# fnothaft/spark-bam

Measured on AMD Instinct MI355X. Metric: compressed BAM GB/s for compute-splits + full-check (whole node, 1/2/4/8 GPU), higher is better.
Workload: dtype u8

## Files before the change

### spark-bam_amd/csrc/sbam_inflate.hip

```cpp
#include <type_traits>

#include "sbam_internal.h"
#include "sbam_resolve_core.h"

namespace sbam {

#define SB_DEV __device__ __forceinline__

enum : int32_t { INF_OK = 0, INF_SHORT = 1, INF_DATA = 2, INF_OVERFLOW = 3 };

constexpr uint32_t kTokPad = 0x7fffu;
constexpr uint32_t kTokDist = 0x8000u;

SB_DEV uint64_t tok_region(int64_t uoff, int64_t b) {
  return (((uint64_t)uoff + 15) & ~15ull) + 32ull * (uint64_t)b;
}
SB_DEV int32_t tok_region_cap(int32_t us) { return (us + 16) / 2; }
SB_DEV uint64_t tok_arena_need(int32_t us) { return ((uint64_t)(2 * us + 32) + 15) & ~15ull; }

constexpr int kDecThreads = 256;
constexpr int kRows = 80;
constexpr int kLitSorted = 0;
constexpr int kClTab = 0;
constexpr int kLensLitRow = 32;
// ... 726 lines not shown
  bool over = false;
  uint32_t code = 0;
  sfor<1, 16>([&](auto I) {
    constexpr int l = decltype(I)::value;
    const uint32_t k = uni(cnt[l]);
    left = 2 * left - (int)k;
    over |= left < 0;
    c.lim[l] = (code + k) << (15 - l);
    c.base[l] = acc - (int32_t)code;
    offs[l] = acc;
    acc += (int32_t)k;
    code = (code + k) << 1;
  });
  c.lim[0] = 0;
  c.base[0] = 0;
  if (over || left != 0) return false;
  int32_t run[16];
  sfor<1, 16>([&](auto I) { run[decltype(I)::value] = 0; });
  for (int c0 = 0; c0 < nsym; c0 += 64) {
    const int s = c0 + lane;
    const uint32_t l = s < nsym ? lens[off + s] : 0u;
    sfor<1, 16>([&](auto I) {
      constexpr int ll = decltype(I)::value;
      const uint64_t m = __ballot(l == (uint32_t)ll);
      const uint32_t below = __builtin_amdgcn_mbcnt_hi((uint32_t)(m >> 32), __builtin_amdgcn_mbcnt_lo((uint32_t)m, 0u));
      if (l == (uint32_t)ll) sorted[off + offs[ll] + run[ll] + (int)below] = (uint16_t)s;
      run[ll] += __popcll(m);
    });
  }
  __syncthreads();
  for (int e = lane; e < (1 << R); e += 64) {
    const uint32_t v = (__builtin_bitreverse32((uint32_t)e) >> (32 - R)) << (15 - R);
    if (v < c.lim[R]) {
      const uint32_t l = canon_len<R>(c, v);
      L.tab[2 * e + DIST] = sym_entry(sorted[off + (int)(v >> (15 - l)) + canon_base<R>(c, l)], l, DIST);
    }
  }
  const uint32_t P0 = c.lim[R] >> (15 - R);
  const int npre = (1 << R) - (int)P0;
  uint16_t *own = reinterpret_cast<uint16_t *>(L.win);
  uint32_t *pinfo = L.win + 256;
  static_assert(wd::kLitSub <= 512 && 256 + 512 <= wd::kWinDw - wd::kScratchDw, "sub-table scratch in the window");
  int next = 0;
  for (int j0 = 0; j0 < npre; j0 += 64) {
    const int j = j0 + lane;
    const uint32_t P = P0 + (uint32_t)j;
    uint32_t sb = 0, sz = 0;
    if (j < npre) {
      sb = canon_len(c, ((P + 1) << (15 - R)) - 1) - R;
      sz = 1u << sb;
    }
    const uint32_t incl = wave_incl_scan(sz);
    const int my = next + (int)(incl - sz);
    if (j < npre && my + (int)sz <= subcap) {
      L.tab[2 * (__builtin_bitreverse32(P) >> (32 - R)) + DIST] =
          (wd::K_SUBP << 8) | sb | ((uint32_t)(4 * (suboff + my)) << 16);
      pinfo[j] = (uint32_t)my | (sb << 16);
      for (uint32_t k = 0; k < sz; k++) own[my + (int)k] = (uint16_t)j;
    }
    next += (int)__shfl(incl, 63);
  }
  __syncthreads();
  if (next <= subcap) {
    for (int e = lane; e < next; e += 64) {
      const int j = own[e];
      const uint32_t info = pinfo[j], sb = info >> 16, P = P0 + (uint32_t)j, k = (uint32_t)e - (info & 0xffffu);
      const uint32_t v = (P << (15 - R)) | ((__builtin_bitreverse32(k) >> (32 - sb)) << (15 - R - sb));
      const uint32_t l = canon_len(c, v);
      L.tab[suboff + e] = sym_entry(sorted[off + (int)(v >> (15 - l)) + canon_base(c, l)], l, DIST);
    }
  }
  __syncthreads();
  return next <= subcap;
}

SB_DEV uint32_t lds_addr(const void *p) {
  return (uint32_t)(uintptr_t)(const __attribute__((address_space(3))) void *)p;
}

typedef const __attribute__((address_space(3))) uint32_t *lds_u32;
SB_DEV lds_u32 win_at(const uint32_t *wp, int pos) {
  uint32_t a;
  asm("v_lshl_add_u32 %0, %1, 2, %2" : "=v"(a) : "v"((uint32_t)pos >> 5), "s"(lds_addr(wp)));
  return reinterpret_cast<lds_u32>((uintptr_t)a);
}
SB_DEV uint32_t tsym(const WaveLds &L, uint32_t lo0, uint32_t hi, int &pos, uint32_t st4, uint32_t &v) {
  using namespace wd;
  const uint32_t lo = __builtin_amdgcn_alignbit(hi, lo0, (uint32_t)pos);
  static_assert(kLitRoot == 9 && kDistRoot == 9, "interleaved 9-bit roots");
  const char *tb = reinterpret_cast<const char *>(L.tab);
  uint32_t e = *reinterpret_cast<const uint32_t *>(tb + (((lo << 3) & 0xff8u) | st4));
  if (((e >> 8) & 0xffu) == K_SUBP)
    e = *reinterpret_cast<const uint32_t *>(tb + (e >> 16) + 4u * __builtin_amdgcn_ubfe(lo, 9u, e));
  const uint32_t n = e & 15u, x = (e >> 4) & 15u;
  v = (e >> 16) + __builtin_amdgcn_ubfe(lo, n, x);
  pos += (int)(n + x);
  return (e >> 8) & 0xffu;
}
SB_DEV uint32_t wsym(const uint32_t *wp, const WaveLds &L, int &pos, uint32_t st4, uint32_t &v) {
  const lds_u32 q = win_at(wp, pos);
  return tsym(L, q[0], q[1], pos, st4, v);
}

struct HBits {
  uint64_t bb;
  int bc, rp, pos;
  SB_DEV void init(const uint32_t *win, int wq, int p) {
    const int rel = p - wq, w = rel >> 5, sh = rel & 31;
    bb = (((uint64_t)uni(win[w]) | ((uint64_t)uni(win[w + 1]) << 32)) >> sh);
    bc = 64 - sh;
    rp = w + 2;
    pos = p;
  }
  SB_DEV uint32_t get(const uint32_t *win, int n) {
    if (bc < 32) {
      bb |= (uint64_t)uni(win[rp]) << bc;
      bc += 32;
      rp++;
    }
    const uint32_t v = (uint32_t)bb & ((1u << n) - 1u);
    bb >>= n;
    bc -= n;
    pos += n;
    return v;
  }
};

SB_DEV void wave_stage(uint32_t *win, const uint32_t *base, int64_t base_dw, int wq_dw, int64_t lim_dw) {
  constexpr int kN = (wd::kWinDw + 255) / 256;
  const int lane = (int)threadIdx.x;
  __syncthreads();
  {
    const int64_t last = lim_dw - 4 - base_dw;
#pragma unroll
    for (int k = 0; k < kN; k++) {
      const int i = lane * 4 + 256 * k;
      if (i < wd::kWinDw) {
        int64_t o = (int64_t)wq_dw + i;
        o = o > last ? last : o;
        __builtin_amdgcn_global_load_lds(base + o, win + 256 * k, 16, 0, 0);
      }
    }
    asm volatile("s_waitcnt vmcnt(0)" ::: "memory");
  }
  __syncthreads();
}
struct SegResult {
  uint32_t tok, byt, exit;
  int stop;
  bool bad;
};

#ifdef SBAM_WAVE_STATS
constexpr int kWaveStats = 40;
__device__ unsigned long long g_wave_stats[kWaveStats];
#define WMARK(slot) do { const uint64_t t_ = __builtin_amdgcn_s_memtime(); ws_[slot] += t_ - wt_; wt_ = t_; } while (0)
#define WADD(slot, v) ws_[slot] += (v)
extern "C" int sbam_debug_wave_stats(unsigned long long *out, int reset) {
  if (hipMemcpyFromSymbol(out, HIP_SYMBOL(g_wave_stats), sizeof(g_wave_stats)) != hipSuccess) return -1;
  if (reset) {
    static const unsigned long long z[kWaveStats] = {0};
    if (hipMemcpyToSymbol(HIP_SYMBOL(g_wave_stats), z, sizeof(z)) != hipSuccess) return -1;
  }
  return 0;
}
#else
#define WMARK(slot) do {} while (0)
#define WADD(slot, v) do {} while (0)
#endif
#ifdef SBAM_WAVE_STATS
#define RMARK(k) do { const uint64_t t_ = __builtin_amdgcn_s_memtime(); rs_[k] += t_ - rt_; rt_ = t_; } while (0)
#else
#define RMARK(k) do {} while (0)
#endif

constexpr int kMaxStored = 64;
constexpr int64_t kTokDone = -2;

SB_DEV bool stored_copy(const uint8_t *__restrict__ d, int64_t a, int dlen, int bitp, int32_t us,
                        uint8_t *__restrict__ ob, int64_t U0, uint32_t *seg) {
  const int lane = (int)threadIdx.x;
  int n = 0, o = 0;
  if ((bitp + 3 + 7) / 8 > dlen) return false;
  bool fin;
  {
    const uint32_t h3 = (uint32_t)d[a + (bitp >> 3)] | (uint32_t)d[a + (bitp >> 3) + 1] << 8;
    const uint32_t hb = (h3 >> (bitp & 7)) & 7u;
    if (((hb >> 1) & 3u) != 0u) return false;
    fin = (hb & 1u) != 0u;
    bitp += 3;
  }
  for (;;) {
    const int byp = (bitp + 7) >> 3;
    if (byp + 4 > dlen || n == kMaxStored) return false;
    const uint32_t len = (uint32_t)d[a + byp] | (uint32_t)d[a + byp + 1] << 8;
    const uint32_t nlen = (uint32_t)d[a + byp + 2] | (uint32_t)d[a + byp + 3] << 8;
    if ((len ^ 0xffffu) != nlen) return false;
    const int dat = byp + 4;
    if (dat + (int)len > dlen) return false;
    if (lane == 0) {
      seg[2 * n] = (uint32_t)o;
      seg[2 * n + 1] = (uint32_t)dat;
    }
    n++;
    o += (int)len;
    if (o > us) return false;
    if (fin) break;
    const int nb = dat + (int)len;
    if (nb >= dlen) return false;
    const uint32_t h3 = d[a + nb];
    if (((h3 >> 1) & 3u) != 0u) return false;
    fin = (h3 & 1u) != 0u;
    bitp = nb * 8 + 3;
  }
  if (o != us) return false;
  __syncthreads();
  for (int j = 0; j < n; j++) {
    const int o0 = (int)seg[2 * j], o1 = j + 1 < n ? (int)seg[2 * j + 2] : us;
    const uint8_t *src = d + a + (int)seg[2 * j + 1] - o0;
    const int c0 = o0 + (int)((16 - ((U0 + o0) & 15)) & 15), c1 = o1 - (int)((U0 + o1) & 15);
    if (c0 + 16 <= c1) {
      int x = c0 + 16 * lane;
      for (; x + 3 * 1024 + 16 <= c1; x += 4 * 1024) {
        const u32x4 v0 = __builtin_nontemporal_load(reinterpret_cast<const u32x4 *>(src + x));
        const u32x4 v1 = __builtin_nontemporal_load(reinterpret_cast<const u32x4 *>(src + x + 1024));
        const u32x4 v2 = __builtin_nontemporal_load(reinterpret_cast<const u32x4 *>(src + x + 2048));
        const u32x4 v3 = __builtin_nontemporal_load(reinterpret_cast<const u32x4 *>(src + x + 3072));
        *reinterpret_cast<u32x4 *>(ob + x) = v0;
        *reinterpret_cast<u32x4 *>(ob + x + 1024) = v1;
        *reinterpret_cast<u32x4 *>(ob + x + 2048) = v2;
        *reinterpret_cast<u32x4 *>(ob + x + 3072) = v3;
      }
      for (; x + 16 <= c1; x += 1024)
        *reinterpret_cast<u32x4 *>(ob + x) = __builtin_nontemporal_load(reinterpret_cast<const u32x4 *>(src + x));
      if (lane < c0 - o0) ob[o0 + lane] = src[o0 + lane];
      if (lane < o1 - c1) ob[c1 + lane] = src[c1 + lane];
    } else {
      for (int x = o0 + lane; x < o1; x += 64) ob[x] = src[x];
    }
  }
  return true;
}

__global__ __launch_bounds__(64, 4) void k_inflate_wave(const uint8_t *__restrict__ d, int64_t D, BlockTable bt,
                                                     TokPool tp, int32_t *__restrict__ status,
                                                     int32_t *__restrict__ found, int32_t *__restrict__ slow,
                                                     unsigned int *nslow) {
  using namespace wd;
  __shared__ __attribute__((aligned(16))) WaveLds L;
  const int lane = (int)threadIdx.x;
  const int64_t b = blockIdx.x;
  const int64_t st0 = bt.start[b];
  const int32_t hs = bt.hsize[b], cs = bt.csize[b], us = bt.usize[b];
  const int32_t dlen = cs - hs - 8;
  if (us == 0 || us < 0 || us > 65536 || dlen < 0 || st0 + hs + dlen > D) {
    if (lane == 0) {
      status[b] = us == 0 ? INF_OK : INF_DATA;
      found[b] = 0;
    }
    return;
  }
  const int64_t a = st0 + hs;
  const int64_t base_dw = (a >> 4) << 2;
  const uint32_t *base = reinterpret_cast<const uint32_t *>(d) + base_dw;
  const int64_t lim_dw = (D + kCompPad) >> 2;
  const int skip = (int)(a - base_dw * 4) * 8;
  const int pend = skip + 8 * dlen;
  uint8_t *reg = tp.main + tok_region(bt.uoff[b], b);
  int32_t tcap = tok_region_cap(us);
  uint8_t *lens = L.lens();
  int pos = skip;
  int out = 0, ntok = 0;
  bool ok = true, stored = false;
#ifdef SBAM_WAVE_STATS
  uint64_t ws_[32] = {0};
  uint64_t wt_ = __builtin_amdgcn_s_memtime();
  const uint64_t wt0_ = wt_;
#endif

  for (bool fin = false; ok && !fin;) {
    int wq = (pos >> 7) << 7;
    wave_stage(L.win, base, base_dw, wq >> 5, lim_dw);
    WMARK(12);
    if (pos + 3 > pend) { ok = false; break; }
    HBits h;
    h.init(L.win, wq, pos);
    fin = h.get(L.win, 1) != 0;
    const uint32_t type = h.get(L.win, 2);
    int hlit = 288, hdist = 32;
    if (type == 1) {
      for (int i = lane; i < 320; i += 64)
        lens[i] = i < 144 ? 8 : i < 256 ? 9 : i < 280 ? 7 : i < 288 ? 8 : 5;
    } else if (type == 2) {
      hlit = (int)h.get(L.win, 5) + 257;
      hdist = (int)h.get(L.win, 5) + 1;
      const int hclen = (int)h.get(L.win, 4) + 4;
      if (hlit > 286 || hdist > 30) { ok = false; break; }
      uint64_t clp = 0;
      for (int i = 0; i < 19; i++)
        if (i < hclen) clp |= (uint64_t)h.get(L.win, 3) << (3 * kClOrder[i]);
      const uint32_t lsym = lane < 19 ? (uint32_t)(clp >> (3 * lane)) & 7u : 0u;
      int left = 1;
      bool over = false;
      uint32_t lim7[8], base7[8], code = 0;
      int acc = 0;
#pragma unroll
      for (int l = 1; l <= 7; l++) {
// ... 374 lines not shown
        if (lane < (nb - nb16) / 2)
          reinterpret_cast<uint16_t *>(nreg + nb16)[lane] = reinterpret_cast<const uint16_t *>(reg + nb16)[lane];
        if (lane == 0) tp.base[b] = (int64_t)at;
        reg = nreg;
        tcap = 1 << 30;
      }
      bool tail = false;
      uint32_t tail_ti = 0, tail_st = 0;
      uint32_t r_lo = 0, r_hi = 0, r_tb = 0;
      if (act) {
        uint32_t start = __shfl_up(nxt, 1);
        if (lane == 0) start = S;
        uint32_t ti = (uint32_t)ntok + (itok - my_tok);
        auto run = [&](uint32_t st, int endp) {
          uint32_t st4 = (st >> 7) & 4u;
          int rp = (int)(st >> 10);
          while (rp < endp) {
            uint32_t v;
            const uint32_t kind = wsym(wp, L, rp, st4, v);
            if (kind == K_SPEC) break;
            st4 = kind == K_LEN ? 4u : 0u;
            *reinterpret_cast<uint16_t *>(reg + 2 * ti) = (uint16_t)v;
            ti++;
          }
        };
        WMARK(24);
        run(start, mode == kModeF ? seg_end : mode == kModeR ? (int)rjP : 0);
        WMARK(25);
        const uint32_t lo = mode == kModeR ? rjs : 0u;
        const uint32_t n = mode == kModeA ? res.tok : mode == kModeR ? res.tok - rjtk : 0u;
        const uint32_t hi = mode == kModeF ? 0u : min(lo + n, (uint32_t)kTR);
        const uint32_t tb = ti - lo;
        r_lo = lo;
        r_hi = hi;
        r_tb = tb;
        static_assert(kTR == 80, "one asm operand per register token dword");
        asm volatile("" : "+v"(tr[0]), "+v"(tr[1]), "+v"(tr[2]), "+v"(tr[3]), "+v"(tr[4]), "+v"(tr[5]), "+v"(tr[6]), "+v"(tr[7]), "+v"(tr[8]), "+v"(tr[9]), "+v"(tr[10]), "+v"(tr[11]), "+v"(tr[12]), "+v"(tr[13]), "+v"(tr[14]), "+v"(tr[15]), "+v"(tr[16]), "+v"(tr[17]), "+v"(tr[18]), "+v"(tr[19]), "+v"(tr[20]), "+v"(tr[21]), "+v"(tr[22]), "+v"(tr[23]), "+v"(tr[24]), "+v"(tr[25]), "+v"(tr[26]), "+v"(tr[27]), "+v"(tr[28]), "+v"(tr[29]), "+v"(tr[30]), "+v"(tr[31]), "+v"(tr[32]), "+v"(tr[33]), "+v"(tr[34]), "+v"(tr[35]), "+v"(tr[36]), "+v"(tr[37]), "+v"(tr[38]), "+v"(tr[39]));
        {
          const uint32_t par = tb & 1u;
          uint8_t *pa = reg + 2 * ((int64_t)ti - (int64_t)lo);
          if (par && lo == 0 && hi > 0) *reinterpret_cast<uint16_t *>(pa) = (uint16_t)tr[0];
          u32x4a *pv = reinterpret_cast<u32x4a *>(pa + 2 * par);
          uint32_t *pw = reinterpret_cast<uint32_t *>(pa + 2 * par);
          auto dw = [&](auto Q) {
            constexpr int q = decltype(Q)::value;
            const uint32_t nx = q + 1 < kTR / 2 ? tr[q + 1 < kTR / 2 ? q + 1 : q] : 0u;
            return par ? __builtin_amdgcn_alignbit(nx, tr[q], 16) : tr[q];
          };
          sfor<0, kTR / 8>([&](auto C) {
            constexpr int c = decltype(C)::value;
            const uint32_t a0 = dw(std::integral_constant<int, 4 * c>{}), a1 = dw(std::integral_constant<int, 4 * c + 1>{});
            const uint32_t a2 = dw(std::integral_constant<int, 4 * c + 2>{}), a3 = dw(std::integral_constant<int, 4 * c + 3>{});
            const uint32_t t0 = par + 8 * c;
            if (t0 >= lo && t0 + 8 <= hi) {
              pv[c] = u32x4a{a0, a1, a2, a3};
            } else if (t0 + 8 > lo && t0 < hi) {
              const uint32_t a[4] = {a0, a1, a2, a3};
#pragma unroll
              for (int k = 0; k < 4; k++) {
                const uint32_t u0 = t0 + 2 * k;
                const bool in0 = u0 >= lo && u0 < hi, in1 = u0 + 1 >= lo && u0 + 1 < hi;
                uint16_t *ph = reinterpret_cast<uint16_t *>(pw + 4 * c + k);
                if (in0 && in1) pw[4 * c + k] = a[k];
                else if (in0) ph[0] = (uint16_t)a[k];
                else if (in1) ph[1] = (uint16_t)(a[k] >> 16);
              }
            }
          });
        }
        WMARK(26);
        WMARK(27);
        tail = mode != kModeF && lo + n > (uint32_t)kTR;
        tail_st = lo <= (uint32_t)kTR ? stR : rjP << 10;
        tail_ti = lo <= (uint32_t)kTR ? tb + kTR : ti;
      }
      if (tail) {
        uint32_t st4 = (tail_st >> 7) & 4u, ti = tail_ti;
        int rp = (int)(tail_st >> 10);
        while (rp < seg_end) {
          uint32_t v;
          const uint32_t kind = wsym(wp, L, rp, st4, v);
          if (kind == K_SPEC) break;
          st4 = kind == K_LEN ? 4u : 0u;
          *reinterpret_cast<uint16_t *>(reg + 2 * ti) = (uint16_t)v;
          ti++;
        }
      }
      (void)r_lo;
      (void)r_hi;
      (void)r_tb;
      WMARK(28);
      out += (int)tot_byt;
      ntok += (int)tot_tok;
      if (f < 64) {
        pos = (int)(uni((uint32_t)__shfl(res.exit, f)) >> 10);
        break;
      }
      S = uni((uint32_t)__shfl(nxt, 63));
    }
  }
  if (ok && out != us) ok = false;
#ifdef SBAM_WAVE_STATS
  ws_[8] = __builtin_amdgcn_s_memtime() - wt0_;
  if (lane == 0)
    for (int i = 0; i < 29; i++) atomicAdd(&g_wave_stats[i], (unsigned long long)ws_[i]);
#endif
  if (lane == 0) {
    if (ok) {
      status[b] = INF_OK;
      found[b] = us;
    } else if (stored) {
      slow[bt.n + atomicAdd(nslow + 3, 1u)] = (int32_t)b;
    } else {
      slow[atomicAdd(nslow, 1u)] = (int32_t)b;
    }
  }
}

__global__ __launch_bounds__(64) void k_inflate_stored(const uint8_t *__restrict__ d, BlockTable bt, TokPool tp,
                                                      uint8_t *__restrict__ out, int32_t *__restrict__ status,
                                                      int32_t *__restrict__ found, int32_t *__restrict__ slow,
                                                      unsigned int *nslow) {
  __shared__ uint32_t seg[2 * kMaxStored];
  const unsigned n = nslow[3];
  for (unsigned i = blockIdx.x; i < n; i += gridDim.x) {
    const int64_t b = slow[bt.n + i];
    const int64_t a = bt.start[b] + bt.hsize[b], U0 = bt.uoff[b];
    const int32_t dlen = bt.csize[b] - bt.hsize[b] - 8, us = bt.usize[b];
    if (stored_copy(d, a, dlen, 0, us, out + U0, U0, seg)) {
      if (threadIdx.x == 0) {
        tp.base[b] = kTokDone;
        status[b] = INF_OK;
        found[b] = us;
      }
    } else if (threadIdx.x == 0) {
      slow[atomicAdd(nslow, 1u)] = (int32_t)b;
    }
    __syncthreads();
  }
}

namespace rs {
constexpr int kSpan = 1024;
constexpr int kFlush = 1024;
}
namespace rc = sbam_resolve;

template <int RB>
struct RingGeom {
  static constexpr uint32_t kRing = 1u << RB, kMask = kRing - 1u, kDw = kRing / 4u, kDwMask = kDw - 1u;
  static constexpr uint32_t kMirror = 8u;
  static constexpr int kNear = (int)kRing - rs::kSpan - 264;
  static_assert(kNear >= rs::kSpan + rs::kFlush + 272, "far sources are in HBM");
  static_assert((int)kRing > rs::kSpan + 260 + rs::kFlush, "slots are flushed before reuse");
};

template <class G>
SB_DEV void ring_or1(uint32_t *ring, uint32_t i, uint32_t w) {
  atomicOr(ring + i, w);
  if (i < G::kMirror) atomicOr(ring + G::kDw + i, w);
}
template <class G>
SB_DEV void ring_or5(uint32_t *ring, uint32_t q, uint32_t w0, uint32_t w1, uint32_t w2, uint32_t w3, uint32_t w4) {
  if (q >= G::kMirror && q + 4u < G::kDw) {
    uint32_t *p = ring + q;
    atomicOr(p + 0, w0);
    atomicOr(p + 1, w1);
    atomicOr(p + 2, w2);
    atomicOr(p + 3, w3);
    atomicOr(p + 4, w4);
  } else {
    ring_or1<G>(ring, q & G::kDwMask, w0);
    ring_or1<G>(ring, (q + 1u) & G::kDwMask, w1);
    ring_or1<G>(ring, (q + 2u) & G::kDwMask, w2);
    ring_or1<G>(ring, (q + 3u) & G::kDwMask, w3);
    ring_or1<G>(ring, (q + 4u) & G::kDwMask, w4);
  }
}

template <int RB>
__global__ __launch_bounds__(64) void k_inflate_resolve(BlockTable bt, uint8_t *__restrict__ out, TokPool pool,
                                                        const int32_t *__restrict__ found,
                                                        const int32_t *__restrict__ list, int32_t *__restrict__ redo,
                                                        unsigned int *__restrict__ nredo) {
  using G = RingGeom<RB>;
  __shared__ __attribute__((aligned(16))) uint32_t ring[G::kDw + G::kMirror];
  __shared__ __attribute__((aligned(16))) uint32_t s_keep[17 * 4];
  uint8_t *ring8 = reinterpret_cast<uint8_t *>(ring);
  const int lane = (int)threadIdx.x;
  for (int i = lane; i < 17 * 4; i += 64) {
    const int n = i >> 2, k = i & 3, nb = n - 4 * k;
    s_keep[i] = nb >= 4 ? ~0u : nb <= 0 ? 0u : (1u << (8 * nb)) - 1u;
  }
  const int64_t b = list ? list[blockIdx.x] : blockIdx.x;
  const int ae = found[b];
  const int64_t tbase = pool.base[b];
  if (ae <= 0 || tbase == kTokDone) return;
  const int64_t U0 = bt.uoff[b];
  uint8_t *ob = out + U0;
  const uint32_t Gr = (uint32_t)U0 & G::kMask;
  const uint16_t *tk =
      reinterpret_cast<const uint16_t *>(tbase >= 0 ? pool.arena + tbase : pool.main + tok_region(U0, b));
  const int F0 = (int)((16 - (U0 & 15)) & 15);
  int F = F0;
  bool head = F0 == 0;
  int Z = -(int)(Gr & 3u);
  int B = 0, tp = 0;
  bool toofar = false;
  uint32_t ta = tk[2 * lane], tb = tk[2 * lane + 1], tn = tk[2 * lane + 2];
  asm volatile("" : "+v"(ta), "+v"(tb), "+v"(tn));
#ifdef SBAM_WAVE_STATS
  uint64_t rs_[8] = {0};
  uint32_t it_ = 0;
  uint64_t itw_ = 0, itl_ = 0;
  uint64_t rt_ = __builtin_amdgcn_s_memtime();
  const uint64_t rt0_ = rt_;
#endif
  while (B < ae) {
    const bool aLit = ta < 256u, aLen = (ta >> 8) == 1u, bLit = tb < 256u, bLen = (tb >> 8) == 1u;
    const int nl = (int)aLit + (int)bLit;
    const int Lm = aLen ? (int)ta - 253 : bLen ? (int)tb - 253 : 0;
    const int d = (int)((aLen ? tb : tn) & 0x7fffu) + 1;
    const int Ln = nl + Lm;
    const int incl = (int)wave_incl_scan((uint32_t)Ln);
    const int ex = incl - Ln;
    const int O = B + ex;
    const bool take = ex < rs::kSpan && O < ae;
    const uint64_t tmask = __ballot(take);
    const int nt = __popcll(tmask);
    const int E = min(B + __builtin_amdgcn_readlane(incl, nt - 1), ae);
    if (E <= B) break;
    const int tp2 = uni(tp + 2 * nt + (int)((__ballot(bLen) >> (nt - 1)) & 1ull));
    {
      const uint32_t z0 = (Gr + (uint32_t)Z) >> 2, z1 = (Gr + (uint32_t)E + 3u) >> 2;
#pragma unroll 1
      for (uint32_t k0 = z0; k0 < z1; k0 += 64u) {
        const uint32_t k = k0 + (uint32_t)lane, i = k & G::kDwMask;
        if (k < z1) {
          ring[i] = 0u;
          if (i < G::kMirror) ring[G::kDw + i] = 0u;
        }
      }
      Z = (int)(z1 * 4u - Gr);
    }
    RMARK(0);
    const int Ll = take ? min(nl, ae - O) : 0;
    if (Ll > 0) {
      const uint32_t lv = aLit ? (ta | (bLit ? tb << 8 : 0u)) : tb;
      const uint32_t x = (Gr + (uint32_t)O) & G::kMask;
      ring8[x] = (uint8_t)lv;
      if (x < 4u * G::kMirror) ring8[G::kRing + x] = (uint8_t)lv;
      if (Ll >= 2) {
        const uint32_t x1 = (x + 1u) & G::kMask;
        ring8[x1] = (uint8_t)(lv >> 8);
        if (x1 < 4u * G::kMirror) ring8[G::kRing + x1] = (uint8_t)(lv >> 8);
      }
    }
    RMARK(1);
    if (!head && B >= F0) {
      if (lane < F0) ob[lane] = ring8[(Gr + (uint32_t)lane) & G::kMask];
      head = true;
    }
    while (B - F >= rs::kFlush) {
      const uint32_t x = (Gr + (uint32_t)(F + 16 * lane)) & G::kMask;
      *reinterpret_cast<uint4 *>(ob + F + 16 * lane) = *reinterpret_cast<const uint4 *>(ring8 + x);
      F += rs::kFlush;
    }
    RMARK(2);
    const int mO = O + (bLen ? nl : 0);
    int Le = (take && Lm > 0) ? min(Lm, ae - mO) : 0;
    const bool tf = Le > 0 && d > mO;
    toofar |= tf;
    Le = tf ? 0 : Le;
    const bool mt = Le > 0;
    const bool far = d > G::kNear;
    const int srcEnd = mO - d + min(Le, d);
    u32x4 pf0 = {0u, 0u, 0u, 0u}, pf1 = {0u, 0u, 0u, 0u};
    if (mt && far) {
      pf0 = __builtin_nontemporal_load(reinterpret_cast<const u32x4 *>(ob + mO - d));
      if (Le > 16) pf1 = __builtin_nontemporal_load(reinterpret_cast<const u32x4 *>(ob + mO - d + 16));
    }
    uint32_t w2, n2;
    __builtin_memcpy(&w2, tk + tp2 + 2 * lane, 4);
    n2 = tk[tp2 + 2 * lane + 2];
    RMARK(3);
    static_assert(G::kNear > rc::kMaxMatch, "a dependent's source is near");
    const bool ind = mt && srcEnd <= B;
    const uint64_t dm = __ballot(mt && !ind);
    uint64_t rem = dm;
    int cut = 0;
    int dsrc = 0, ddst = -1;
    auto lay_out = [&]() {
      int s = -(1 << 30), o = -1;
      int t = 0, c = cut;
      cut = 0;
      uint64_t m = rem;
      do {
        const int k = 63 - __clzll((long long)m);
        const uint64_t bit = 1ull << k;
        m &= ~bit;
        const int mk = __builtin_amdgcn_readlane(mO, k), dk = __builtin_amdgcn_readlane(d, k),
                  lk = __builtin_amdgcn_readlane(Le, k);
        const int r = s - mk;
        const bool hit = rc::hop_hits(s, mk, lk);
        const int left = lk - c, n = min(left, 64 - t);
        const int jj = lane - t + (left - n);
        const bool act = (uint32_t)(lane - t) < (uint32_t)n;
        int rf = r, jf = jj;
        if (lk > dk) {
          int dv = dk;
          asm volatile("" : "+v"(dv));
          rf = rc::period_offset(r, dv);
          jf = rc::period_offset(jj, dv);
        }
        const int base = mk - dk;
        s = act ? base + jf : hit ? base + rf : s;
        o = act ? mk + jj : o;
        if (n == left) rem &= ~bit;
        else if (t < 64) cut = c + n;
        t += n;
        c = 0;
      } while (m);
      dsrc = s;
      ddst = o;
    };
    if (rem) lay_out();
    if (ind) {
      int done = 0, deff = d;
      while (done < Le) {
#ifdef SBAM_WAVE_STATS
        it_++;
#endif
        const int n = min(min(Le - done, 16), deff);
        const int src = mO + done - deff;
        const uint4 km = *reinterpret_cast<const uint4 *>(s_keep + 4 * n);
        uint32_t v0, v1, v2, v3;
        if (far) {
          if (done >= 32) {
            const u32x4 x = __builtin_nontemporal_load(reinterpret_cast<const u32x4 *>(ob + src));
            v0 = x.x; v1 = x.y; v2 = x.z; v3 = x.w;
            asm volatile("" : "+v"(v0), "+v"(v1), "+v"(v2), "+v"(v3));
          } else {
            const u32x4 x = done == 0 ? pf0 : pf1;
            v0 = x.x; v1 = x.y; v2 = x.z; v3 = x.w;
            asm volatile("" : "+v"(v0), "+v"(v1), "+v"(v2), "+v"(v3));
          }
        } else {
          const uint32_t xs = (Gr + (uint32_t)src) & G::kMask, qs = xs >> 2, ss = xs & 3u;
          const uint32_t *p = ring + qs;
          const uint32_t s0 = p[0], s1 = p[1], s2 = p[2], s3 = p[3], s4 = p[4];
          v0 = __builtin_amdgcn_alignbyte(s1, s0, ss);
          v1 = __builtin_amdgcn_alignbyte(s2, s1, ss);
          v2 = __builtin_amdgcn_alignbyte(s3, s2, ss);
          v3 = __builtin_amdgcn_alignbyte(s4, s3, ss);
        }
        v0 &= km.x;
        v1 &= km.y;
        v2 &= km.z;
        v3 &= km.w;
        const uint32_t xd = (Gr + (uint32_t)(mO + done)) & G::kMask, qd = xd >> 2, s8 = (xd & 3u) * 8u;
        const uint64_t a01 = ((uint64_t)v1 << 32 | v0) << s8, a12 = ((uint64_t)v2 << 32 | v1) << s8,
                       a23 = ((uint64_t)v3 << 32 | v2) << s8, a34 = (uint64_t)v3 << s8;
        ring_or5<G>(ring, qd, (uint32_t)a01, (uint32_t)(a01 >> 32), (uint32_t)(a12 >> 32), (uint32_t)(a23 >> 32),
                    (uint32_t)(a34 >> 32));
        done += n;
        if (n == deff && deff < 16) deff *= 2;
      }
    }
#ifdef SBAM_WAVE_STATS
    {
      uint32_t mx = it_, sm = it_;
      for (int o = 32; o >= 1; o >>= 1) {
        mx = max(mx, (uint32_t)__shfl_xor((int)mx, o));
        sm += (uint32_t)__shfl_xor((int)sm, o);
      }
      itw_ += mx;
      itl_ += sm;
      it_ = 0;
    }
#endif
    RMARK(4);
    for (;;) {
      if (ddst >= 0) {
        const uint8_t v = ring8[(Gr + (uint32_t)dsrc) & G::kMask];
        const uint32_t x = (Gr + (uint32_t)ddst) & G::kMask;
        ring8[x] = v;
        if (x < 4u * G::kMirror) ring8[G::kRing + x] = v;
      }
      if (!rem) break;
      lay_out();
    }
    RMARK(5);
    B = E;
    asm volatile("" : "+v"(w2), "+v"(n2));
    ta = w2 & 0xffffu;
    tb = w2 >> 16;
    tn = n2;
    RMARK(6);
#ifdef SBAM_WAVE_STATS
    rs_[7]++;
#endif
    tp = tp2;
  }
  if (!head) {
    if (lane < min(F0, ae)) ob[lane] = ring8[(Gr + (uint32_t)lane) & G::kMask];
  }
  if (ae > F0) {
    const int Ft = F + ((ae - F) & ~15);
    for (int p = F + 16 * lane; p < Ft; p += rs::kFlush)
      *reinterpret_cast<uint4 *>(ob + p) = *reinterpret_cast<const uint4 *>(ring8 + ((Gr + (uint32_t)p) & G::kMask));
    if (Ft + lane < ae) ob[Ft + lane] = ring8[(Gr + (uint32_t)(Ft + lane)) & G::kMask];
  }
  if (__ballot(toofar) != 0 && lane == 0 && redo) redo[atomicAdd(nredo, 1u)] = (int32_t)b;
#ifdef SBAM_WAVE_STATS
  const uint64_t tot_ = __builtin_amdgcn_s_memtime() - rt0_;
  if (lane == 0) {
    for (int i = 0; i < 8; i++) atomicAdd(&g_wave_stats[32 + i], (unsigned long long)rs_[i]);
    atomicAdd(&g_wave_stats[31], (unsigned long long)tot_);
    atomicAdd(&g_wave_stats[29], (unsigned long long)itw_);
    atomicAdd(&g_wave_stats[30], (unsigned long long)itl_);
  }
#endif
}

__global__ void k_first_error(const int32_t *__restrict__ status, int64_t n, unsigned long long *first_err) {
  const int64_t i = (int64_t)blockIdx.x * blockDim.x + threadIdx.x;
  if (i < n && status[i] != INF_OK) atomicMin(first_err, (unsigned long long)i);
}

hipError_t launch_first_error(const int32_t *status, int64_t n, unsigned long long *first_err, hipStream_t s) {
  if (n == 0) return hipSuccess;
  hipLaunchKernelGGL(k_first_error, dim3((unsigned)((n + 255) / 256)), dim3(256), 0, s, status, n, first_err);
  return hipGetLastError();
}


hipError_t launch_inflate_decode(const uint8_t *d, int64_t D, BlockTable bt, TokPool tok, uint8_t *out,
                                 int32_t *status, int32_t *found, int32_t *slow, unsigned int *counters,
                                 hipStream_t s) {
  (void)hipMemsetAsync(counters, 0, 4 * sizeof(unsigned int), s);
  if (bt.n == 0) return hipSuccess;
  hipLaunchKernelGGL(k_inflate_wave, dim3((unsigned)bt.n), dim3(64), 0, s, d, D, bt, tok, status, found, slow,
                     counters + 0);
  hipLaunchKernelGGL(k_inflate_stored, dim3(4096), dim3(64), 0, s, d, bt, tok, out, status, found, slow,
                     counters + 0);
  hipLaunchKernelGGL(k_inflate_slow, dim3(256), dim3(kDecThreads), 0, s, d, D, bt, tok, slow, counters + 0, status,
                     found, counters + 1);
  return hipGetLastError();
}

hipError_t launch_inflate_resolve(BlockTable bt, uint8_t *out, TokPool tok, const int32_t *found,
                                  const int32_t *list, int64_t nlist, int32_t *redo, unsigned int *nredo,
                                  hipStream_t s) {
  const int64_t n = list ? nlist : bt.n;
  if (n == 0) return hipSuccess;
  hipLaunchKernelGGL(k_inflate_resolve<12>, dim3((unsigned)n), dim3(64), 0, s, bt, out, tok, found, list, redo, nredo);
  return hipGetLastError();
}

hipError_t launch_inflate_redo(const uint8_t *d, int64_t D, BlockTable bt, TokPool tok, const int32_t *list,
                               unsigned int *counters, int32_t *status, int32_t *found, hipStream_t s) {
  (void)hipMemsetAsync(counters + 1, 0, sizeof(unsigned int), s);
  hipLaunchKernelGGL(k_inflate_slow, dim3(256), dim3(kDecThreads), 0, s, d, D, bt, tok, list, counters + 2, status,
                     found, counters + 1);
  return hipGetLastError();
}

}
```

### spark-bam_amd/csrc/sbam_resolve_core.h

```cpp
#pragma once
#include <stdint.h>

#if defined(__HIPCC__)
#include <hip/hip_runtime.h>
#define SBAM_RS_HD __host__ __device__ inline __attribute__((always_inline))
#else
#define SBAM_RS_HD inline
#endif

namespace sbam_resolve {

constexpr int kMaxMatch = 258;

SBAM_RS_HD int period_offset(int r, int d) { return r < d ? r : (int)((uint32_t)r % (uint32_t)d); }

SBAM_RS_HD int collapsed_source(int mO, int d, int j) { return mO - d + period_offset(j, d); }

SBAM_RS_HD bool hop_hits(int s, int mOk, int Lek) { return (uint32_t)(s - mOk) < (uint32_t)Lek; }

SBAM_RS_HD int sweep_hop(int s, int mOk, int dk, int Lek) {
  return hop_hits(s, mOk, Lek) ? collapsed_source(mOk, dk, s - mOk) : s;
}

SBAM_RS_HD int sweep(int s, const int *mO, const int *d, const int *Le, int n) {
  for (int k = n - 1; k >= 0; k--) s = sweep_hop(s, mO[k], d[k], Le[k]);
  return s;
}

}
```

Baseline: 88.57.

## Software-pipeline inflate resolve: decode next step and prefetch far matches early

Restructures the resolve loop into a two-stage software pipeline with double-buffered step registers. While the current step is being laid out, the next step's token header is decoded and its far match source is prefetched from HBM when that source has already been flushed. This aims to hide global-memory latency for far back-references behind the current step's LDS work. It adds register pressure and extra per-step control flow, and relies on the stored-mark check to keep prefetches from reading bytes that have not yet been written.

```diff
diff --git a/spark-bam_amd/csrc/sbam_inflate.hip b/spark-bam_amd/csrc/sbam_inflate.hip
--- a/spark-bam_amd/csrc/sbam_inflate.hip
+++ b/spark-bam_amd/csrc/sbam_inflate.hip
@@ -902,7 +902,7 @@
 };
 
 #ifdef SBAM_WAVE_STATS
-constexpr int kWaveStats = 40;
+constexpr int kWaveStats = 42;
 __device__ unsigned long long g_wave_stats[kWaveStats];
 #define WMARK(slot) do { const uint64_t t_ = __builtin_amdgcn_s_memtime(); ws_[slot] += t_ - wt_; wt_ = t_; } while (0)
 #define WADD(slot, v) ws_[slot] += (v)
@@ -1583,6 +1583,8 @@
   static constexpr uint32_t kMirror = 8u;
   static constexpr int kNear = (int)kRing - rs::kSpan - 264;
   static_assert(kNear >= rs::kSpan + rs::kFlush + 272, "far sources are in HBM");
+  static_assert(rs::kFlush % 16 == 0, "the stored mark is a 16-B boundary");
+  static_assert(kNear >= rc::kMaxMatch, "a far match never reads its own output");
   static_assert((int)kRing > rs::kSpan + 260 + rs::kFlush, "slots are flushed before reuse");
 };
 
@@ -1609,6 +1611,41 @@
   }
 }
 
+struct ResLane {
+  int O, Ll;
+  uint32_t lv;
+  int mO, d, Le;
+};
+
+SB_DEV bool resolve_head(uint32_t ta, uint32_t tb, uint32_t tn, int B, int ae, ResLane &s, int &E, int &ntok,
+                         bool &toofar) {
+  const bool aLit = ta < 256u, aLen = (ta >> 8) == 1u, bLit = tb < 256u, bLen = (tb >> 8) == 1u;
+  const int nl = (int)aLit + (int)bLit;
+  const int Lm = aLen ? (int)ta - 253 : bLen ? (int)tb - 253 : 0;
+  const int d = (int)((aLen ? tb : tn) & 0x7fffu) + 1;
+  const int Ln = nl + Lm;
+  const int incl = (int)wave_incl_scan((uint32_t)Ln);
+  const int ex = incl - Ln;
+  const int O = B + ex;
+  const bool take = ex < rs::kSpan && O < ae;
+  const uint64_t tmask = __ballot(take);
+  const int nt = __popcll(tmask);
+  E = min(B + __builtin_amdgcn_readlane(incl, nt - 1), ae);
+  if (E <= B) return false;
+  ntok = uni(2 * nt + (int)((__ballot(bLen) >> (nt - 1)) & 1ull));
+  s.O = O;
+  s.Ll = take ? min(nl, ae - O) : 0;
+  s.lv = aLit ? (ta | (bLit ? tb << 8 : 0u)) : tb;
+  const int mO = O + (bLen ? nl : 0);
+  const int Le = (take && Lm > 0) ? min(Lm, ae - mO) : 0;
+  const bool tf = Le > 0 && d > mO;
+  toofar |= tf;
+  s.mO = mO;
+  s.d = d;
+  s.Le = tf ? 0 : Le;
+  return true;
+}
+
 template <int RB>
 __global__ __launch_bounds__(64) void k_inflate_resolve(BlockTable bt, uint8_t *__restrict__ out, TokPool pool,
                                                         const int32_t *__restrict__ found,
@@ -1636,32 +1673,36 @@
   int F = F0;
   bool head = F0 == 0;
   int Z = -(int)(Gr & 3u);
-  int B = 0, tp = 0;
   bool toofar = false;
-  uint32_t ta = tk[2 * lane], tb = tk[2 * lane + 1], tn = tk[2 * lane + 2];
-  asm volatile("" : "+v"(ta), "+v"(tb), "+v"(tn));
+  struct StepRegs {
+    ResLane f;
+    u32x4 pf0, pf1;
+    bool pre;
+  } ra, rb;
+  ra.pf0 = ra.pf1 = rb.pf0 = rb.pf1 = u32x4{0u, 0u, 0u, 0u};
+  ra.pre = rb.pre = false;
+  int B = 0, E = 0, tp = 0;
+  bool have;
+  {
+    uint32_t ta = tk[2 * lane], tb = tk[2 * lane + 1], tn = tk[2 * lane + 2];
+    int ntok = 0;
+    have = resolve_head(ta, tb, tn, 0, ae, ra.f, E, ntok, toofar);
+    tp = ntok;
+  }
+  uint32_t w2, n2;
+  __builtin_memcpy(&w2, tk + tp + 2 * lane, 4);
+  n2 = tk[tp + 2 * lane + 2];
 #ifdef SBAM_WAVE_STATS
-  uint64_t rs_[8] = {0};
+  uint64_t rs_[10] = {0};
   uint32_t it_ = 0;
   uint64_t itw_ = 0, itl_ = 0;
   uint64_t rt_ = __builtin_amdgcn_s_memtime();
   const uint64_t rt0_ = rt_;
 #endif
-  while (B < ae) {
-    const bool aLit = ta < 256u, aLen = (ta >> 8) == 1u, bLit = tb < 256u, bLen = (tb >> 8) == 1u;
-    const int nl = (int)aLit + (int)bLit;
-    const int Lm = aLen ? (int)ta - 253 : bLen ? (int)tb - 253 : 0;
-    const int d = (int)((aLen ? tb : tn) & 0x7fffu) + 1;
-    const int Ln = nl + Lm;
-    const int incl = (int)wave_incl_scan((uint32_t)Ln);
-    const int ex = incl - Ln;
-    const int O = B + ex;
-    const bool take = ex < rs::kSpan && O < ae;
-    const uint64_t tmask = __ballot(take);
-    const int nt = __popcll(tmask);
-    const int E = min(B + __builtin_amdgcn_readlane(incl, nt - 1), ae);
-    if (E <= B) break;
-    const int tp2 = uni(tp + 2 * nt + (int)((__ballot(bLen) >> (nt - 1)) & 1ull));
+  auto step = [&](StepRegs &c, StepRegs &x) __attribute__((always_inline)) -> bool {
+    ResLane &cur = c.f, &nx = x.f;
+    u32x4 &pf0 = c.pf0, &pf1 = c.pf1, &q0 = x.pf0, &q1 = x.pf1;
+    const bool pre = c.pre;
     {
       const uint32_t z0 = (Gr + (uint32_t)Z) >> 2, z1 = (Gr + (uint32_t)E + 3u) >> 2;
 #pragma unroll 1
@@ -1675,19 +1716,20 @@
       Z = (int)(z1 * 4u - Gr);
     }
     RMARK(0);
-    const int Ll = take ? min(nl, ae - O) : 0;
-    if (Ll > 0) {
-      const uint32_t lv = aLit ? (ta | (bLit ? tb << 8 : 0u)) : tb;
-      const uint32_t x = (Gr + (uint32_t)O) & G::kMask;
+    if (cur.Ll > 0) {
+      const uint32_t lv = cur.lv;
+      const uint32_t x = (Gr + (uint32_t)cur.O) & G::kMask;
       ring8[x] = (uint8_t)lv;
       if (x < 4u * G::kMirror) ring8[G::kRing + x] = (uint8_t)lv;
-      if (Ll >= 2) {
+      if (cur.Ll >= 2) {
         const uint32_t x1 = (x + 1u) & G::kMask;
         ring8[x1] = (uint8_t)(lv >> 8);
         if (x1 < 4u * G::kMirror) ring8[G::kRing + x1] = (uint8_t)(lv >> 8);
       }
     }
     RMARK(1);
+    asm volatile("" : "+v"(pf0), "+v"(pf1), "+v"(w2), "+v"(n2));
+    RMARK(6);
     if (!head && B >= F0) {
       if (lane < F0) ob[lane] = ring8[(Gr + (uint32_t)lane) & G::kMask];
       head = true;
@@ -1698,22 +1740,35 @@
       F += rs::kFlush;
     }
     RMARK(2);
-    const int mO = O + (bLen ? nl : 0);
-    int Le = (take && Lm > 0) ? min(Lm, ae - mO) : 0;
-    const bool tf = Le > 0 && d > mO;
-    toofar |= tf;
-    Le = tf ? 0 : Le;
+    const int mO = cur.mO, d = cur.d, Le = cur.Le;
     const bool mt = Le > 0;
     const bool far = d > G::kNear;
     const int srcEnd = mO - d + min(Le, d);
-    u32x4 pf0 = {0u, 0u, 0u, 0u}, pf1 = {0u, 0u, 0u, 0u};
-    if (mt && far) {
-      pf0 = __builtin_nontemporal_load(reinterpret_cast<const u32x4 *>(ob + mO - d));
-      if (Le > 16) pf1 = __builtin_nontemporal_load(reinterpret_cast<const u32x4 *>(ob + mO - d + 16));
-    }
-    uint32_t w2, n2;
-    __builtin_memcpy(&w2, tk + tp2 + 2 * lane, 4);
-    n2 = tk[tp2 + 2 * lane + 2];
+    if (__ballot(mt && far && !pre) != 0) {
+      if (mt && far && !pre) {
+        pf0 = __builtin_nontemporal_load(reinterpret_cast<const u32x4 *>(ob + mO - d));
+        if (Le > 16) pf1 = __builtin_nontemporal_load(reinterpret_cast<const u32x4 *>(ob + mO - d + 16));
+      }
+      asm volatile("" : "+v"(pf0), "+v"(pf1));
+    }
+    RMARK(9);
+    int E2 = E, tp2 = tp;
+    bool have2 = false, pre2 = false;
+    if (E < ae) {
+      int ntok = 0;
+      have2 = resolve_head(w2 & 0xffffu, w2 >> 16, n2, E, ae, nx, E2, ntok, toofar);
+      if (have2) {
+        const int mark = rc::stored_mark(head, F);
+        pre2 = nx.Le > 0 && nx.d > G::kNear && rc::far_source_stored(nx.mO, nx.d, nx.Le, mark);
+        if (pre2) {
+          q0 = __builtin_nontemporal_load(reinterpret_cast<const u32x4 *>(ob + nx.mO - nx.d));
+          if (nx.Le > 16) q1 = __builtin_nontemporal_load(reinterpret_cast<const u32x4 *>(ob + nx.mO - nx.d + 16));
+        }
+        tp2 = tp + ntok;
+        __builtin_memcpy(&w2, tk + tp2 + 2 * lane, 4);
+        n2 = tk[tp2 + 2 * lane + 2];
+      }
+    }
     RMARK(3);
     static_assert(G::kNear > rc::kMaxMatch, "a dependent's source is near");
     const bool ind = mt && srcEnd <= B;
@@ -1756,6 +1811,7 @@
       ddst = o;
     };
     if (rem) lay_out();
+    RMARK(8);
     if (ind) {
       int done = 0, deff = d;
       while (done < Le) {
@@ -1822,17 +1878,18 @@
       lay_out();
     }
     RMARK(5);
+    x.pre = pre2;
     B = E;
-    asm volatile("" : "+v"(w2), "+v"(n2));
-    ta = w2 & 0xffffu;
-    tb = w2 >> 16;
-    tn = n2;
-    RMARK(6);
+    E = E2;
+    tp = tp2;
 #ifdef SBAM_WAVE_STATS
     rs_[7]++;
 #endif
-    tp = tp2;
-  }
+    return have2;
+  };
+  if (have)
+    while (step(ra, rb) && step(rb, ra)) {
+    }
   if (!head) {
     if (lane < min(F0, ae)) ob[lane] = ring8[(Gr + (uint32_t)lane) & G::kMask];
   }
@@ -1847,6 +1904,8 @@
   const uint64_t tot_ = __builtin_amdgcn_s_memtime() - rt0_;
   if (lane == 0) {
     for (int i = 0; i < 8; i++) atomicAdd(&g_wave_stats[32 + i], (unsigned long long)rs_[i]);
+    atomicAdd(&g_wave_stats[40], (unsigned long long)rs_[8]);
+    atomicAdd(&g_wave_stats[41], (unsigned long long)rs_[9]);
     atomicAdd(&g_wave_stats[31], (unsigned long long)tot_);
     atomicAdd(&g_wave_stats[29], (unsigned long long)itw_);
     atomicAdd(&g_wave_stats[30], (unsigned long long)itl_);
diff --git a/spark-bam_amd/csrc/sbam_resolve_core.h b/spark-bam_amd/csrc/sbam_resolve_core.h
--- a/spark-bam_amd/csrc/sbam_resolve_core.h
+++ b/spark-bam_amd/csrc/sbam_resolve_core.h
@@ -27,4 +27,8 @@
   return s;
 }
 
+SBAM_RS_HD int stored_mark(bool head, int F) { return head ? F : 0; }
+
+SBAM_RS_HD bool far_source_stored(int mO, int d, int Le, int mark) { return mO - d + Le <= mark; }
+
 }
```

Result: no change. 89.16 (median of 6 runs) (+0.7%).
